# Seasandwpy/viso

Measured on AMD Instinct MI355X. Metric: stereo frames/sec at 1242x375 grey, 1/2/4/8 GPUs; pose RMSE vs reference, higher is better.
Workload: dtype f64

## Files before the change

### viso_amd/csrc/common.hpp

```cpp
#pragma once

#include <hip/hip_runtime.h>

#include <cstddef>
#include <cstdint>
#include <cstdio>

namespace viso {

constexpr int kLevels = 4;
constexpr int kHalfPatch = 4;
constexpr int kPatch = 64;
constexpr int kMaxWidth = 4096;

struct PyrGeom {
    int w[kLevels], h[kLevels];
    size_t off[kLevels];
    size_t bytes;
    size_t slot;
};

inline PyrGeom make_geom(int w, int h) {
    PyrGeom g{};
    size_t off = 0;
// ... 36 lines not shown
    return ((const __attribute__((address_space(1))) uint8_t*)p)[i];
}
__device__ inline uint8_t ld_global_u8_off(const uint8_t* base, uint32_t off) {
    return ((const __attribute__((address_space(1))) uint8_t*)base)[off];
}
__device__ inline int ld_u8_or0(const uint8_t* p, long long n, long long i) {
    const bool in = i >= 0 && i < n;
    const int v = ld_global_u8(p, in ? i : 0);
    return in ? v : 0;
}
__device__ inline uint8_t ld_lds_u8(const uint8_t* p, int i) {
    return ((const __attribute__((address_space(3))) uint8_t*)p)[i];
}
__device__ inline void st_lds_u8(uint8_t* p, int i, uint8_t v) {
    ((__attribute__((address_space(3))) uint8_t*)p)[i] = v;
}

__device__ inline double sample_px(const uint8_t* __restrict__ img, int w, int h, double x,
                                   double y) {
    const long long n = (long long)w * (long long)h;
    const bool finite = (x > -1e9 && x < 1e9 && y > -1e9 && y < 1e9);
    long long base = finite ? (long long)(int)y * (long long)w + (long long)(int)x : -(1LL << 40);
    double d0 = (double)ld_u8_or0(img, n, base);
    double d1 = (double)ld_u8_or0(img, n, base + 1);
    double d2 = (double)ld_u8_or0(img, n, base + w);
    double d3 = (double)ld_u8_or0(img, n, base + w + 1);
    double xx = x - floor(x);
    double yy = y - floor(y);
    return double((1 - xx) * (1 - yy) * d0 + xx * (1 - yy) * d1 + (1 - xx) * yy * d2 +
                  xx * yy * d3);
}

__device__ inline void gradient_px(const uint8_t* __restrict__ img, int w, int h, double u,
                                   double v, double& gx, double& gy) {
    gx = 0.5 * (sample_px(img, w, h, u + 1, v) - sample_px(img, w, h, u - 1, v));
    gy = 0.5 * (sample_px(img, w, h, u, v + 1) - sample_px(img, w, h, u, v - 1));
}

__device__ inline double wave_tree_sum(double v) {
#pragma unroll
    for (int off = 1; off < 64; off <<= 1) v = v + __shfl_xor(v, off, 64);
    return v;
}

template <int CTRL>
__device__ inline double dpp_f64(double v) {
    const long long b = __double_as_longlong(v);
    const int lo = __builtin_amdgcn_mov_dpp((int)(b & 0xffffffffLL), CTRL, 0xF, 0xF, true);
    const int hi = __builtin_amdgcn_mov_dpp((int)(b >> 32), CTRL, 0xF, 0xF, true);
    return __longlong_as_double(((long long)hi << 32) | (unsigned int)lo);
}

__device__ inline int wave_id() { return __builtin_amdgcn_readfirstlane((int)(threadIdx.x >> 6)); }

__device__ inline double uniform_f64(double v) {
    const long long b = __double_as_longlong(v);
    const int lo = __builtin_amdgcn_readfirstlane((int)(b & 0xffffffffLL));
    const int hi = __builtin_amdgcn_readfirstlane((int)(b >> 32));
    return __longlong_as_double(((long long)hi << 32) | (unsigned int)lo);
}

__device__ inline double readlane_f64(double v, int lane) {
    const long long b = __double_as_longlong(v);
    const int lo = __builtin_amdgcn_readlane((int)(b & 0xffffffffLL), lane);
    const int hi = __builtin_amdgcn_readlane((int)(b >> 32), lane);
    return __longlong_as_double(((long long)hi << 32) | (unsigned int)lo);
}

__device__ inline void permlane16_swap_f64(double a, double b, double& ra, double& rb) {
    const long long x = __double_as_longlong(a), y = __double_as_longlong(b);
    const auto lo = __builtin_amdgcn_permlane16_swap((unsigned)(x & 0xffffffffLL),
                                                     (unsigned)(y & 0xffffffffLL), false, false);
    const auto hi = __builtin_amdgcn_permlane16_swap((unsigned)(x >> 32), (unsigned)(y >> 32), false,
                                                     false);
    ra = __longlong_as_double(((long long)hi[0] << 32) | lo[0]);
    rb = __longlong_as_double(((long long)hi[1] << 32) | lo[1]);
}

__device__ inline void permlane32_swap_f64(double a, double b, double& ra, double& rb) {
    const long long x = __double_as_longlong(a), y = __double_as_longlong(b);
    const auto lo = __builtin_amdgcn_permlane32_swap((unsigned)(x & 0xffffffffLL),
                                                     (unsigned)(y & 0xffffffffLL), false, false);
    const auto hi = __builtin_amdgcn_permlane32_swap((unsigned)(x >> 32), (unsigned)(y >> 32), false,
                                                     false);
    ra = __longlong_as_double(((long long)hi[0] << 32) | lo[0]);
    rb = __longlong_as_double(((long long)hi[1] << 32) | lo[1]);
}

__device__ inline double wave_tree_sum_dpp(double v) {
    v = v + dpp_f64<0xB1>(v);
    v = v + dpp_f64<0x4E>(v);
    v = v + dpp_f64<0x141>(v);
    v = v + dpp_f64<0x140>(v);
    double a, b;
    permlane16_swap_f64(v, v, a, b);
    v = a + b;
    permlane32_swap_f64(v, v, a, b);
    return a + b;
}

__device__ inline double dsel(bool c, double a, double b) { return c ? a : b; }

__device__ inline void wave_tree_sum3(double a, double b, double c, double& ra, double& rb, double& rc) {
    const int lane = threadIdx.x & 63;
    const bool b0 = lane & 1, b1 = lane & 2, b2 = lane & 4, b3 = lane & 8;
    const double p = (b0 ? b : a) + dpp_f64<0xB1>(b0 ? a : b);
    const double q = (b0 ? 0.0 : c) + dpp_f64<0xB1>(b0 ? c : 0.0);
    double v = (b1 ? q : p) + dpp_f64<0x4E>(b1 ? p : q);
    const double r4 = dpp_f64<0x114>(v), l4 = dpp_f64<0x104>(v);
    v = v + dsel(b2, r4, l4);
    v = v + dpp_f64<0x128>(v);
    double x, y;
    permlane16_swap_f64(v, v, x, y);
    v = x + y;
    permlane32_swap_f64(v, v, x, y);
    v = x + y;
    ra = readlane_f64(v, 0);
    rb = readlane_f64(v, 1);
    rc = readlane_f64(v, 2);
}

__device__ inline void wave_tree_sum3_desc(double a, double b, double c, double& ra, double& rb, double& rc) {
    const int lane = threadIdx.x & 63;
    const bool b2 = lane & 4, b3 = lane & 8;
    double x, y;
    permlane32_swap_f64(a, b, x, y);
    const double ab = x + y;
    permlane32_swap_f64(c, c, x, y);
    const double cc = x + y;
    permlane16_swap_f64(ab, cc, x, y);
    double v = x + y;
    v = v + dpp_f64<0x128>(v);
    v = v + dpp_f64<0x124>(v);
    v = v + dpp_f64<0x4E>(v);
    v = v + dpp_f64<0xB1>(v);
    ra = readlane_f64(v, 0);
    rb = readlane_f64(v, 32);
    rc = readlane_f64(v, 16);
}


template <int CTRL>
__device__ inline double dpp_or0(double v) {
    return dpp_f64<CTRL>(v);
}

__device__ inline double swizzle_xor16_f64(double v) {
    const long long b = __double_as_longlong(v);
    const int lo = __builtin_amdgcn_ds_swizzle((int)(b & 0xffffffffLL), 0x401F);
    const int hi = __builtin_amdgcn_ds_swizzle((int)(b >> 32), 0x401F);
    return __longlong_as_double(((long long)hi << 32) | (unsigned int)lo);
}

__device__ inline double reduce_scatter_28(const double* v, int* value_index) {
    const int lane = threadIdx.x & 63;
    const bool b0 = lane & 1, b1 = lane & 2, b2 = lane & 4, b3 = lane & 8, b4 = lane & 16;
    double a[14];
#pragma unroll
    for (int k = 0; k < 14; ++k) {
        const double send = dsel(b0, v[k], v[14 + k]);
        const double keep = dsel(b0, v[14 + k], v[k]);
        a[k] = keep + dpp_f64<0xB1>(send);
    }
    double c[7];
#pragma unroll
    for (int k = 0; k < 7; ++k) {
        const double send = dsel(b1, a[k], a[7 + k]);
        const double keep = dsel(b1, a[7 + k], a[k]);
        c[k] = keep + dpp_f64<0x4E>(send);
    }
    double d[4];
#pragma unroll
    for (int k = 0; k < 4; ++k) {
        const double hi = k < 3 ? c[4 + k] : 0.0;
        const double send = dsel(b2, c[k], hi);
        const double keep = dsel(b2, hi, c[k]);
        const double recv = dsel(b2, dpp_f64<0x114>(send), dpp_f64<0x104>(send));
        d[k] = keep + recv;
    }
    double e[2];
#pragma unroll
    for (int k = 0; k < 2; ++k) {
        const double send = dsel(b3, d[k], d[2 + k]);
        const double keep = dsel(b3, d[2 + k], d[k]);
        const double recv = dpp_f64<0x128>(send);
        e[k] = keep + recv;
    }
    double ra, rb;
    permlane16_swap_f64(e[0], e[1], ra, rb);
    double f = ra + rb;
    permlane32_swap_f64(f, f, ra, rb);
    f = ra + rb;
    *value_index = (b0 ? 14 : 0) + (b1 ? 7 : 0) + (b2 ? 4 : 0) + (b3 ? 2 : 0) + (b4 ? 1 : 0);
    const int local = (b2 ? 4 : 0) + (b3 ? 2 : 0) + (b4 ? 1 : 0);
    if (local >= 7) *value_index = -1;
    return f;
}

__device__ inline double reduce_scatter_28_desc(const double* v, int* value_index) {
    const int lane = threadIdx.x & 63;
    const bool b0 = lane & 1, b1 = lane & 2, b2 = lane & 4, b3 = lane & 8, b4 = lane & 16, b5 = lane & 32;
    double a[14];
#pragma unroll
    for (int k = 0; k < 14; ++k) {
        double ra, rb;
        permlane32_swap_f64(v[k], v[14 + k], ra, rb);
        a[k] = ra + rb;
    }
    double c[7];
#pragma unroll
    for (int k = 0; k < 7; ++k) {
        double ra, rb;
        permlane16_swap_f64(a[k], a[7 + k], ra, rb);
        c[k] = ra + rb;
    }
    double d[4];
#pragma unroll
    for (int k = 0; k < 4; ++k) {
        const double hi = k < 3 ? c[4 + k] : 0.0;
        const double send = dsel(b3, c[k], hi);
        const double keep = dsel(b3, hi, c[k]);
        const double recv = dpp_f64<0x128>(send);
        d[k] = keep + recv;
    }
    double e[2];
#pragma unroll
    for (int k = 0; k < 2; ++k) {
        const double send = dsel(b2, d[k], d[2 + k]);
        const double keep = dsel(b2, d[2 + k], d[k]);
        const double recv = dsel(b2, dpp_f64<0x114>(send), dpp_f64<0x104>(send));
        e[k] = keep + recv;
    }
    const double send = dsel(b1, e[0], e[1]);
    const double keep = dsel(b1, e[1], e[0]);
    double f = keep + dpp_f64<0x4E>(send);
    f = f + dpp_f64<0xB1>(f);
    const int local = (b3 ? 4 : 0) + (b2 ? 2 : 0) + (b1 ? 1 : 0);
    *value_index = (b0 || local >= 7) ? -1 : (b5 ? 14 : 0) + (b4 ? 7 : 0) + local;
    return f;
}

template <int CTRL>
__device__ inline float dpp_f32(float v) {
    return __int_as_float(__builtin_amdgcn_mov_dpp(__float_as_int(v), CTRL, 0xF, 0xF, true));
}

__device__ inline void permlane16_swap_f32(float a, float b, float& ra, float& rb) {
    const auto r = __builtin_amdgcn_permlane16_swap((unsigned)__float_as_int(a), (unsigned)__float_as_int(b),
                                                    false, false);
    ra = __int_as_float((int)r[0]);
    rb = __int_as_float((int)r[1]);
}

__device__ inline void permlane32_swap_f32(float a, float b, float& ra, float& rb) {
    const auto r = __builtin_amdgcn_permlane32_swap((unsigned)__float_as_int(a), (unsigned)__float_as_int(b),
                                                    false, false);
    ra = __int_as_float((int)r[0]);
    rb = __int_as_float((int)r[1]);
}

__device__ inline float reduce_scatter_28_f32(const float* v, int* value_index) {
    const int lane = threadIdx.x & 63;
    const bool b0 = lane & 1, b1 = lane & 2, b2 = lane & 4, b3 = lane & 8, b4 = lane & 16;
    float a[14];
#pragma unroll
    for (int k = 0; k < 14; ++k) {
        const float send = b0 ? v[k] : v[14 + k];
        const float keep = b0 ? v[14 + k] : v[k];
        a[k] = keep + dpp_f32<0xB1>(send);
    }
    float c[7];
#pragma unroll
    for (int k = 0; k < 7; ++k) {
        const float send = b1 ? a[k] : a[7 + k];
        const float keep = b1 ? a[7 + k] : a[k];
        c[k] = keep + dpp_f32<0x4E>(send);
    }
    float d[4];
#pragma unroll
    for (int k = 0; k < 4; ++k) {
        const float hi = k < 3 ? c[4 + k] : 0.0f;
        const float send = b2 ? c[k] : hi;
        const float keep = b2 ? hi : c[k];
        const float r4 = dpp_f32<0x114>(send), l4 = dpp_f32<0x104>(send);
        const float recv = b2 ? r4 : l4;
        d[k] = keep + recv;
    }
    float e[2];
#pragma unroll
    for (int k = 0; k < 2; ++k) {
        const float send = b3 ? d[k] : d[2 + k];
        const float keep = b3 ? d[2 + k] : d[k];
        e[k] = keep + dpp_f32<0x128>(send);
    }
    float ra, rb;
    permlane16_swap_f32(e[0], e[1], ra, rb);
    float f = ra + rb;
    permlane32_swap_f32(f, f, ra, rb);
    f = ra + rb;
    *value_index = (b0 ? 14 : 0) + (b1 ? 7 : 0) + (b2 ? 4 : 0) + (b3 ? 2 : 0) + (b4 ? 1 : 0);
    const int local = (b2 ? 4 : 0) + (b3 ? 2 : 0) + (b4 ? 1 : 0);
    if (local >= 7) *value_index = -1;
    return f;
}

__device__ inline void wave_tree_sum3_f32(float a, float b, float c, float& ra, float& rb, float& rc) {
// ... 68 lines not shown
```

### viso_amd/csrc/direct.hip

```cpp
#include <algorithm>
#include <cstring>

#include "device_math.hpp"
#include "direct_solve.hpp"
#include "kernels.hpp"

#ifdef VISO_PROBE
constexpr int kPRing = 4096;
constexpr int kPSt = 16;
__device__ unsigned long long g_plog[kPRing][kPSt];
__device__ unsigned long long g_pexit[kPRing];
constexpr int kPRingB = 512;
__device__ unsigned long long g_pblk[kPRingB][256][4];
__device__ unsigned long long g_pwave[kPRingB][256][16];
#ifdef VISO_PROBE_PT
constexpr int kPtRing = 128, kPtBlocks = 32, kPtStamps = 5;
__device__ unsigned long long g_ppt[kPtRing][kPtBlocks][16][kPtStamps];
#define PPT(k)                                                                                       \
    do {                                                                                             \
        if (blockIdx.x < kPtBlocks && (threadIdx.x & 63) == 0)                                       \
            g_ppt[a.probe_seq & (kPtRing - 1)][blockIdx.x][threadIdx.x >> 6][(k)] =                  \
                __builtin_amdgcn_s_memrealtime();                                                    \
    } while (0)
#endif
#define PROBE_DECL()                                \
    __shared__ unsigned long long pst[kPSt];        \
    const unsigned long long probe_t0 = __builtin_amdgcn_s_memrealtime()
#define PST(k)                                                                       \
    do {                                                                             \
        if (blockIdx.x == 0 && (threadIdx.x & 63) == 0) pst[(k)] = __builtin_amdgcn_s_memrealtime(); \
    } while (0)
#else
#define PROBE_DECL()
#define PST(k)
#endif
#ifndef VISO_PROBE_PT
#define PPT(k) ((void)0)
#endif

namespace viso {

namespace {

constexpr int kSums = 28;
#ifndef VISO_DIRECT_WAVES
#define VISO_DIRECT_WAVES 12
#endif
constexpr int kWaves = VISO_DIRECT_WAVES;
constexpr int kThreads = kWaves * 64;
constexpr int kRigWaves = 16;
constexpr int kRigThreads = kRigWaves * 64;
constexpr int kMaxTiles = 256;
constexpr int kMaxTile = kMaxMapPoints / kMaxTiles;

inline int map_tile(int n, int groups) {
    int t = (n + groups - 1) / groups;
    return t < 1 ? 1 : (t > kMaxTile ? kMaxTile : t);
}
constexpr int kStats = 50;
constexpr int kStateStride = 8;
constexpr int kHdrBg = 1 << 17;

struct FramePair {
    FrameDev last;
    FrameDev cur;
    const double* pose_last;
};

struct LevelPair {
    const uint8_t* last;
    const uint8_t* cur;
    const double* pose_last;
};

__device__ inline LevelPair level_pair(const FramePair& fp, int lv) {
    return LevelPair{fp.last.l[lv], fp.cur.l[lv], fp.pose_last};
}

struct DirectArgs {
    FramePair fp;
    PyrDev g;
    Intrinsics K;
    const double* points;
    int n;
    const double* pose_seed;
    int level;
    int tile;
    int n_tiles;
    int split;
    DirectScratch s;
    double* stats;
    double* pose_out;
    double* log;
    int log_index;
    double* log_host;
    double* prev_log_host;
    int merged;
    int probe_seq;
    FramePair prev;
    double* prev_pose_out;
    double* prev_log;
    int prev_log_index;
    int* ready;
    int* prev_ready;
    double* flog;
};

__device__ inline void store_frame_pose(double* dst, const double* pose, int* ready) {
#pragma unroll
    for (int k = 0; k < 12; ++k) __hip_atomic_store(dst + k, pose[k], __ATOMIC_RELAXED, __HIP_MEMORY_SCOPE_AGENT);
    if (ready) {
        asm volatile("s_waitcnt vmcnt(0)" ::: "memory");
        __hip_atomic_store(ready, 1, __ATOMIC_RELAXED, __HIP_MEMORY_SCOPE_AGENT);
    }
}

__device__ inline void log_pose(double* log, double* log_host, int index, const double* pose) {
    if (!log || index < 0) return;
    for (int k = 0; k < 12; ++k) log[12 * (size_t)index + k] = pose[k];
    if (log_host)
        for (int k = 0; k < 12; ++k)
            __hip_atomic_store(log_host + 12 * (size_t)index + k, pose[k], __ATOMIC_RELAXED, __HIP_MEMORY_SCOPE_SYSTEM);
}

__device__ inline void log_frame(double* flog, int index, const SolveLds& L) {
    if (!flog || index < 0) return;
    flog[4 * (size_t)index + 0] = (double)L.ngood;
    flog[4 * (size_t)index + 1] = L.cost;
}

__device__ inline void tile_range(const DirectArgs& a, int b, int* first, int* cnt) {
    if (a.split) {
        const int f = (int)(((long long)b * a.n) / a.n_tiles);
        *first = f;
        *cnt = (int)(((long long)(b + 1) * a.n) / a.n_tiles) - f;
    } else {
        *first = b * a.tile;
        *cnt = a.tile;
    }
}

__device__ inline void d_pixel_d_xi(const Intrinsics& K, const double* pose, const double* P,
                                    double scale, double* J) {
    double Pc[3];
    mat3_vec(pose, P, Pc);
    Pc[0] = Pc[0] + pose[9];
    Pc[1] = Pc[1] + pose[10];
    Pc[2] = Pc[2] + pose[11];
    const double x = Pc[0], y = Pc[1], z = Pc[2];
    const double fx = K.fx * scale, fy = K.fy * scale;
    const double zz = z * z, xy = x * y;
    J[0] = fx / z;
    J[1] = 0;
    J[2] = -fx * x / zz;
    J[3] = -fx * xy / zz;
    J[4] = fx + fx * x * x / zz;
    J[5] = -fx * y / z;
    J[6] = 0;
    J[7] = fy / z;
    J[8] = -fy * y / zz;
    J[9] = -fy - fy * y * y / zz;
    J[10] = fy * xy / zz;
// ... 673 lines not shown
    const double xx = uc - floor(uc), yy = vc - floor(vc);
    const double w00 = (1 - xx) * (1 - yy), w10 = xx * (1 - yy), w01 = (1 - xx) * yy, w11 = xx * yy;
    const bool shared = cls == kClsShared;
    if (valid) {
        sp.v[j][k] = q;
        if (k == 0) {
            double2* v2 = reinterpret_cast<double2*>(&sp.v[j][12]);
            v2[0] = make_double2(shared ? w00 : uc, shared ? w10 : vc);
            v2[1] = make_double2(w01, w11);
            *reinterpret_cast<int4*>(sp.cls[j]) = make_int4(cls, fu, fv, 0);
        }
    }
    __builtin_amdgcn_fence(__ATOMIC_RELEASE, "workgroup");
    if (valid && k == 0) __hip_atomic_store(&sp.ready[j], 1, __ATOMIC_RELAXED, __HIP_MEMORY_SCOPE_WORKGROUP);
}

constexpr unsigned kSrcHere = 0xffffffffu;

template <bool FAST, bool LV16 = false, int W = kWaves>
__device__ void direct_tile_pf(const DirectArgs& a, const LevelPair& fp, int lv, const double* cur_pose, int b,
                               const PfLds& pf, bool merged, double* part, int* good, double* s_pts,
                               int* s_good, int* s_cnt = nullptr, double* s_qt = nullptr,
                               unsigned src_in = kSrcHere, SpLds* sp = nullptr) {
    const int wave = wave_id(), lane = threadIdx.x & 63;
    int first, T;
    tile_range(a, b, &first, &T);
    int good_cnt = 0;
    const unsigned src_lanes = FAST ? 0u : src_in != kSrcHere ? src_in : factored_sources();
    const bool sp_on = !FAST && W == kWaves && sp && s_cnt && T > kSpPoints - kSpHelpers && T <= kSpPoints;
    if (sp_on && wave >= kSpPoints) {
        __builtin_amdgcn_s_setprio(3);
        scalar_pass(a, lv, cur_pose, pf, first, T, wave - kSpPoints, *sp);
        __builtin_amdgcn_s_setprio(1);
    }
    for (int local = wave; local < T; local += W) {
        const int i = first + local;
        double f = 0.0;
        int idx = -1;
        bool ok = false;
        if (i < a.n) {
            RefSample r;
            if (merged) {
                merged_ref(a, fp, lv, pf, local, r);
                if (!FAST) ref_finish(r);
            } else if (!FAST) {
                pf_ref(pf, local, r);
            } else {
                r.P[0] = pf.P[local][0];
                r.P[1] = pf.P[local][1];
                r.P[2] = pf.P[local][2];
                r.ur = pf.ur[local];
                r.vr = pf.vr[local];
                r.ok = pf.ok[local] != 0;
                const uint32_t t = pf.taps[local][lane];
                r.t0 = (int)(t & 0xff);
                r.t1 = (int)((t >> 8) & 0xff);
                r.t2 = (int)((t >> 16) & 0xff);
                r.t3 = (int)(t >> 24);
            }
            CurWin cw;
            cw.x0 = pf.cw[local][0];
            cw.y0 = pf.cw[local][1];
            cw.on = pf.cw[local][2] != 0;
            if (FAST) {
                float ff = 0.0f;
                if (r.ok) {
                    const uint32_t t = (uint32_t)r.t0 | ((uint32_t)r.t1 << 8) | ((uint32_t)r.t2 << 16) |
                                       ((uint32_t)r.t3 << 24);
                    const float lval = (LV16 && !merged) ? (float)pf.lv16[local][lane] : fast_lval(t, r.ur, r.vr);
                    ok = direct_point_fast(a, fp, lv, cur_pose, r.P, lval, pf.win[local], cw, &ff, &idx);
                }
                f = (double)ff;
            } else if (sp_on) {
                ok = direct_point_sp(a, fp, lv, r, pf.win[local], cw, *sp, local, &f, &idx, src_lanes);
            } else {
                ok = direct_point_rs(a, fp, lv, cur_pose, r, pf.win[local], cw, &f, &idx, src_lanes,
                                     s_qt ? s_qt + 12 * wave : nullptr);
            }
        }
        if (!ok) {
            if (lane < kSums) s_pts[local * kSums + lane] = 0.0;
        } else if ((!FAST || lane < 32) && idx >= 0) {
            s_pts[local * kSums + idx] = f;
        }
        good_cnt += ok ? 1 : 0;
    }
    if (lane == 0 && good_cnt) atomicAdd(s_good, good_cnt);
#ifdef VISO_PROBE
    if (threadIdx.x == 0 && blockIdx.x < 256) g_pblk[a.probe_seq & (kPRingB - 1)][blockIdx.x][2] = __builtin_amdgcn_s_memrealtime();
    if (lane == 0 && blockIdx.x < 256 && wave < 15)
        g_pwave[a.probe_seq & (kPRingB - 1)][blockIdx.x][wave] = __builtin_amdgcn_s_memrealtime();
#endif
    if (s_cnt && T <= 16) {
        const int nw = T < W ? T : W;
        if (wave >= nw) return;
        int prev = 0;
        if (lane == 0)
            prev = __hip_atomic_fetch_add(s_cnt, 1, __ATOMIC_ACQ_REL, __HIP_MEMORY_SCOPE_WORKGROUP);
        prev = __builtin_amdgcn_readfirstlane(prev);
        if (prev != nw - 1) return;
        __builtin_amdgcn_fence(__ATOMIC_ACQUIRE, "workgroup");
        if (lane < kSums) {
            double v[16];
#pragma unroll
            for (int j = 0; j < 16; ++j) v[j] = j < T ? s_pts[j * kSums + lane] : 0.0;
#pragma unroll
            for (int st = 1; st < 16; st <<= 1)
#pragma unroll
                for (int j = 0; j < 16; j += 2 * st) v[j] = v[j] + v[j + st];
            double r = v[0] + 0.0;
            r = r + 0.0;
            part[(size_t)lane * kMaxTiles + b] = r;
        }
        if (lane == 0) good[b] = __hip_atomic_load(s_good, __ATOMIC_RELAXED, __HIP_MEMORY_SCOPE_WORKGROUP);
#ifdef VISO_PROBE
        if (lane == 0 && blockIdx.x < 256)
            g_pwave[a.probe_seq & (kPRingB - 1)][blockIdx.x][15] = __builtin_amdgcn_s_memrealtime();
#endif
        return;
    }
    __syncthreads();
    for (int k = wave; k < kSums; k += W) {
        const double v = lane < T ? s_pts[lane * kSums + k] : 0.0;
        const double r = wave_tree_sum_dpp(v);
        if (lane == 0) part[(size_t)k * kMaxTiles + b] = r;
    }
    if (threadIdx.x == 0) good[b] = *s_good;
    __syncthreads();
}

__device__ inline void state_to_pose(const double* st, double* pose) {
    double q[4] = {st[0], st[1], st[2], st[3]};
    quat_to_matrix(q, pose);
    pose[9] = st[4];
    pose[10] = st[5];
    pose[11] = st[6];
}


__device__ inline void load_partials(const double* __restrict__ part, const int* __restrict__ good,
                                     int n_tiles, double* v, int& gg) {
    const int t = threadIdx.x;
    if (t < n_tiles) {
#pragma unroll
        for (int k = 0; k < kSums; ++k) v[k] = part[(size_t)k * kMaxTiles + t];
        gg = good[t];
    } else {
#pragma unroll
        for (int k = 0; k < kSums; ++k) v[k] = 0.0;
        gg = 0;
    }
}

__device__ inline void reduce_partials(const double* v, int gg, SolveLds& L) {
    const int t = threadIdx.x, wave = t >> 6, lane = t & 63;
    if (t < 256) {
        int idx;
        const double f = reduce_scatter_28(v, &idx);
        if (lane < 32 && idx >= 0) L.red[wave][idx] = f;
        const int g = wave_sum_int(gg);
        if (lane == 0) L.g[wave] = g;
    }
    __syncthreads();
    if (t < kSums) L.S[t] = (L.red[0][t] + L.red[1][t]) + (L.red[2][t] + L.red[3][t]);
    if (t == 0) L.ngood = (L.g[0] + L.g[1]) + (L.g[2] + L.g[3]);
    __syncthreads();
}

__device__ inline void lds_barrier() { asm volatile("s_waitcnt lgkmcnt(0)\n\ts_barrier" ::: "memory"); }

template <bool FAST>
__device__ void solve_continue(const DirectArgs& a, const FramePair& fpair, int lv, SolveLds& L,
                               double* stats, double* s_pose, double* s_pts, int* s_good, PfLds& pf) {
    const int t = threadIdx.x, wave = t >> 6;
    double* part = a.s.cont_part + (size_t)blockIdx.x * kMaxTiles * kSums;
    int* good = a.s.cont_good + (size_t)blockIdx.x * kMaxTiles;
    const LevelPair fp = level_pair(fpair, lv);
    for (int iter = 1; iter < 100 && L.cont; ++iter) {
        if (t == 0) state_to_pose(L.state, s_pose);
        __syncthreads();
        double pose[12];
#pragma unroll
        for (int k = 0; k < 12; ++k) pose[k] = s_pose[k];
        for (int b = 0; b < a.n_tiles; ++b) {
            if (t == 0) *s_good = 0;
            prefetch_tile(a, lv, b, pose, fpair.pose_last, true, wave, kWaves, pf, &fpair);
            __syncthreads();
            direct_tile_pf<FAST>(a, fp, lv, pose, b, pf, false, part, good, s_pts, s_good);
        }
        __threadfence_block();
        __syncthreads();
        double v[kSums];
        int gg = 0;
        if (t < 256) load_partials(part, good, a.n_tiles, v, gg);
        reduce_partials(v, gg, L);
        if (wave == 0) {
            if (FAST)
                solve_wave0_ldlt(L, iter, stats);
            else
                solve_wave0(L, iter, stats);
        }
        __syncthreads();
    }
}

__device__ inline void prefetch_point(const DirectArgs& a, int lv, int i, bool solve, int sl,
                                      RefSample& r, CurWin& cw) {
    ref_issue(a, level_pair(a.fp, lv), lv, i, r);
    double pred[12];
    if (!solve) {
        for (int k = 0; k < 12; ++k) pred[k] = a.pose_seed[k];
    } else {
        double sp[7];
        for (int k = 0; k < 7; ++k) sp[k] = a.s.state[sl * kStateStride + k];
        state_to_pose(sp, pred);
    }
    double up, vp;
    project_px(pred, a.K, r.P, kScale[lv], up, vp);
    win_issue(a.fp.cur.l[lv], a.g.w[lv], a.g.h[lv], up, vp, cw);
}

__device__ inline void after_solve(const DirectArgs& a, bool merged, SolveLds& L, double* s_last,
                                   double* s_pose) {
    if (merged) {
        state_to_pose(L.state, s_last);
        if (blockIdx.x == 0) {
            for (int k = 0; k < 7; ++k) a.s.state[kLevels * kStateStride + k] = L.state[k];
            if (a.prev_pose_out) store_frame_pose(a.prev_pose_out, s_last, a.prev_ready);
            log_pose(a.prev_log, a.prev_log_host, a.prev_log_index, s_last);
            log_frame(a.flog, a.prev_log_index, L);
        }
        double q[4];
        quat_from_matrix(s_last, q);
        for (int k = 0; k < 4; ++k) L.state[k] = q[k];
        L.state[4] = s_last[9];
        L.state[5] = s_last[10];
        L.state[6] = s_last[11];
    }
    state_to_pose(L.state, s_pose);
}

template <bool FAST, bool SP = false>
__global__ __launch_bounds__(kThreads, 4) void direct_level_kernel(const double* __restrict__ pre_part,
                                                                 const int* __restrict__ pre_good, int pre_hdr,
                                                                 DirectArgs a) {
    PROBE_DECL();
    __builtin_amdgcn_s_setprio(1);
    __shared__ SolveLds L;
    __shared__ double s_pose[12];
    __shared__ double s_last[12];
    __shared__ double s_pts[kMaxTile * kSums];
    __shared__ int s_good;
    __shared__ int s_cnt;
    __shared__ int s_arrive;
    __shared__ PfLds s_pf;
#ifndef VISO_NO_QT
    __shared__ __attribute__((aligned(16))) double s_qt[FAST ? 2 : kWaves * 12];
    double* const qt = FAST ? nullptr : s_qt;
#else
    double* const qt = nullptr;
#endif
    __shared__ __attribute__((aligned(16))) SpLds s_sp;
    const int lv = a.level;
    const bool merged = a.merged && lv == kLevels - 1;
    const int prev = lv + 1;
    const bool solve = prev < kLevels || merged;
    const int sl = merged ? 0 : prev;
    const int t = threadIdx.x, wave = t >> 6, lane = t & 63;
    const bool tiles = lv >= 0 && (int)blockIdx.x < a.n_tiles;
    double v[kSums];
    int gg = 0;
    if (((pre_hdr >> 16) & 1) && t < 256) load_partials(pre_part, pre_good, pre_hdr & 0xffff, v, gg);
    const bool pf_wave = !solve || (wave & 3) != 0;
    double st[7];
    if (t == 256 || (solve && tiles && pf_wave)) {
        if (!solve) {
            quat_from_matrix(a.pose_seed, st);
            st[4] = a.pose_seed[9];
            st[5] = a.pose_seed[10];
            st[6] = a.pose_seed[11];
        } else {
#pragma unroll
            for (int k = 0; k < 7; ++k) st[k] = a.s.state[sl * kStateStride + k];
        }
    }
    if (t == 0) {
        s_arrive = 0;
        s_good = 0;
        s_cnt = 0;
#ifdef VISO_PROBE
        for (int k = 0; k < kPSt; ++k) pst[k] = 0;
        pst[0] = probe_t0;
        if (blockIdx.x < 256) g_pblk[a.probe_seq & (kPRingB - 1)][blockIdx.x][0] = probe_t0;
#endif
    }
    if (SP && t >= kThreads - kSpPoints) s_sp.ready[kThreads - 1 - t] = 0;
    lds_barrier();

    if (t == 256) {
        for (int k = 0; k < 7; ++k) {
            L.state[k] = st[k];
            L.best[k] = st[k];
        }
        L.cost = 0.0;
        L.last_cost = 0.0;
        L.cont = 0;
        asm volatile("s_waitcnt lgkmcnt(0)" ::: "memory");
        atomicAdd(&s_arrive, 1);
    }
    if (solve && t < 256) {
        int idx;
        const double f = reduce_scatter_28(v, &idx);
        if (lane < 32 && idx >= 0) L.red[wave][idx] = f;
        const int g = wave_sum_int(gg);
        if (lane == 0) L.g[wave] = g;
        asm volatile("s_waitcnt lgkmcnt(0)" ::: "memory");
        if (lane == 0) atomicAdd(&s_arrive, 1);
    }
    if (wave == 0) PST(1);

    const bool solver = solve && wave == 0;
    if (tiles && pf_wave) {
        double pred[12];
        if (!solve) {
            for (int k = 0; k < 12; ++k) pred[k] = a.pose_seed[k];
        } else {
            state_to_pose(st, pred);
        }
        const int first = solve ? wave - (wave >> 2) - 1 : wave;
        const int stride = solve ? kWaves - kWaves / 4 : kWaves;
        prefetch_tile(a, lv, blockIdx.x, pred, merged ? pred : a.fp.pose_last, true, first, stride, s_pf);
#ifdef VISO_PROBE
        asm volatile("s_waitcnt vmcnt(0) lgkmcnt(0)" ::: "memory");
        if (blockIdx.x == 0 && lane == 0) atomicMax(&pst[9], __builtin_amdgcn_s_memrealtime());
#endif
    }

    if (solver) {
        __builtin_amdgcn_s_setprio(3);
        while (__hip_atomic_load(&s_arrive, __ATOMIC_RELAXED, __HIP_MEMORY_SCOPE_WORKGROUP) < 5)
            __builtin_amdgcn_s_sleep(1);
        if (lane < kSums) L.S[lane] = (L.red[0][lane] + L.red[1][lane]) + (L.red[2][lane] + L.red[3][lane]);
        if (lane == 0) L.ngood = (L.g[0] + L.g[1]) + (L.g[2] + L.g[3]);
        PST(2);
        double* stp = (a.stats && blockIdx.x == 0) ? a.stats + (size_t)kStats * sl : nullptr;
#ifdef VISO_PROBE
        unsigned long long stamps[5] = {probe_t0, probe_t0, probe_t0, probe_t0, probe_t0};
        if (FAST)
            solve_wave0_ldlt(L, 0, stp, stamps);
        else
            solve_wave0(L, 0, stp, stamps);
        if (blockIdx.x == 0 && lane == 0)
            for (int k = 0; k < 4; ++k) pst[3 + k] = stamps[k];
        if (blockIdx.x == 0 && lane == 0) pst[12] = stamps[4];
#else
        if (FAST)
            solve_wave0_ldlt(L, 0, stp);
        else
            solve_wave0(L, 0, stp);
#endif
        PST(7);
        __builtin_amdgcn_s_setprio(1);
    }
    if (!solve && wave == 0 && lane == 0) {
        while (__hip_atomic_load(&s_arrive, __ATOMIC_RELAXED, __HIP_MEMORY_SCOPE_WORKGROUP) < 1)
            __builtin_amdgcn_s_sleep(1);
    }
    if (wave == 0 && lane == 0 && !L.cont) after_solve(a, merged, L, s_last, s_pose);
    const unsigned src_lanes = FAST ? 0u : factored_sources();
    __syncthreads();
    if (__builtin_expect(solve && L.cont, 0)) {
        double* stp = (a.stats && blockIdx.x == 0) ? a.stats + (size_t)kStats * sl : nullptr;
        solve_continue<FAST>(a, merged ? a.prev : a.fp, sl, L, stp, s_pose, s_pts, &s_good, s_pf);
        if (t == 0) {
            after_solve(a, merged, L, s_last, s_pose);
            s_good = 0;
        }
        __syncthreads();
        if (tiles) {
            double pose[12];
#pragma unroll
            for (int k = 0; k < 12; ++k) pose[k] = s_pose[k];
            prefetch_tile(a, lv, blockIdx.x, pose, merged ? s_last : a.fp.pose_last, true, wave, kWaves, s_pf);
        }
        __syncthreads();
    }
    if (wave == 0) PST(8);
#ifdef VISO_PROBE
    if (t == 0 && blockIdx.x < 256) g_pblk[a.probe_seq & (kPRingB - 1)][blockIdx.x][1] = __builtin_amdgcn_s_memrealtime();
#endif
    const int out = lv >= 0 ? lv : kLevels;
    if (blockIdx.x == 0 && t == 0 && !merged) {
        for (int k = 0; k < 7; ++k) a.s.state[out * kStateStride + k] = L.state[k];
        if (lv < 0 && a.pose_out) {
            store_frame_pose(a.pose_out, s_pose, a.ready);
            log_pose(a.log, a.log_host, a.log_index, s_pose);
            log_frame(a.flog, a.log_index, L);
        }
    }
    if (blockIdx.x == 0 && t == 0 && merged)
        for (int k = 0; k < 7; ++k) a.s.state[lv * kStateStride + k] = L.state[k];
    if (tiles) {
        LevelPair fp = level_pair(a.fp, lv);
        if (merged) fp.pose_last = s_last;
        double pose[12];
#pragma unroll
        for (int k = 0; k < 12; ++k) pose[k] = s_pose[k];
        direct_tile_pf<FAST>(a, fp, lv, pose, blockIdx.x, s_pf, merged, a.s.part + (size_t)lv * kMaxTiles * kSums,
                       a.s.good + lv * kMaxTiles, s_pts, &s_good, &s_cnt, qt, src_lanes,
                       SP ? &s_sp : nullptr);
    }
#ifdef VISO_PROBE
    __syncthreads();
    const unsigned long long t_exit = __builtin_amdgcn_s_memrealtime();
    const int slot = a.probe_seq & (kPRing - 1);
    if (t == 0 && blockIdx.x < 256) g_pblk[a.probe_seq & (kPRingB - 1)][blockIdx.x][3] = t_exit;
    if (blockIdx.x == 0 && t == 0) {
        pst[11] = t_exit;
        pst[15] = (unsigned long long)(lv + 1) | ((unsigned long long)merged << 8) |
                  ((unsigned long long)a.n_tiles << 16);
        for (int k = 0; k < kPSt; ++k) g_plog[slot][k] = pst[k];
    }
#endif
}

constexpr int kRigTiles = kMaxTiles;

__device__ __host__ inline int rig_reduce_waves(int n_tiles) { return n_tiles <= 64 ? 1 : n_tiles <= 128 ? 2 : 4; }

struct RigCamArgs {
    DirectArgs d;
    const double* Ad;
    double E[12];
};

struct RigArgs {
    RigCamArgs cam[kMaxRigCams];
    int n_cams;
    int tile_off[kMaxRigCams + 1];
    int level;
    double* state;
    const double* seed;
    double* stats;
    double* pose_out;
    double* log;
    int log_index;
    double* cam_last;
    int merged;
    double* prev_pose_out;
    double* prev_log;
    int prev_log_index;
};

__device__ inline void rig_compose(const double* E, const double* T, double* out) {
#pragma unroll
    for (int i = 0; i < 3; ++i) {
#pragma unroll
        for (int j = 0; j < 3; ++j)
            out[3 * i + j] = (E[3 * i] * T[j] + E[3 * i + 1] * T[3 + j]) + E[3 * i + 2] * T[6 + j];
        out[9 + i] = ((E[3 * i] * T[9] + E[3 * i + 1] * T[10]) + E[3 * i + 2] * T[11]) + E[9 + i];
    }
}

__device__ inline int rig_camera(const RigArgs& ra, int b) {
    int c = 0;
#pragma unroll
    for (int k = 1; k < kMaxRigCams; ++k) {
        const int off = ra.tile_off[k];
        if (k < ra.n_cams && b >= off) c = k;
    }
    return c;
}

__device__ inline void rig_contrib(int q, double (*red)[kSums], const double* Ad, double* sM, double* con) {
    const int lane = threadIdx.x & 63;
    if (q > 1 && lane < kSums) {
        const double v = q == 2 ? red[0][lane] + red[1][lane]
                                : (red[0][lane] + red[1][lane]) + (red[2][lane] + red[3][lane]);
        red[0][lane] = v;
    }
    asm volatile("s_waitcnt lgkmcnt(0)" ::: "memory");
    const double* S = red[0];
    if (lane < 36) {
        const int i = lane / 6, j = lane - 6 * (lane / 6);
        double m = 0.0;
#pragma unroll
        for (int k = 0; k < 6; ++k) {
            const int a = i < k ? i : k, bb = i < k ? k : i;
            const double h = S[a * 6 - (a * (a - 1)) / 2 + (bb - a)];
            m = k == 0 ? h * Ad[j] : m + h * Ad[6 * k + j];
        }
        sM[lane] = m;
    }
    asm volatile("s_waitcnt lgkmcnt(0)" ::: "memory");
// ... 632 lines not shown
```

### viso_amd/csrc/direct_solve.hpp

```cpp
#pragma once

#include "common.hpp"
#include "device_math.hpp"


namespace viso {

constexpr int kSolveSums = 28;
constexpr int kSolveStateStride = 8;

struct SolveLds {
    double red[4][kSolveSums];
    double S[kSolveSums];
    int g[4];
    int ngood;
    double state[kSolveStateStride], best[kSolveStateStride];
    double cost, last_cost;
    int cont;
};

#define SPROBE(k)                                                   \
    do {                                                            \
        if (stamps) stamps[(k)] = __builtin_amdgcn_s_memrealtime(); \
    } while (0)

__device__ __attribute__((always_inline)) inline void solve_finish(SolveLds& L, const double* update, double h, int iter, double* stats,
                                    unsigned long long* stamps) {
    const int lane = threadIdx.x & 63;
    const bool in = lane < 36;
    const int ngood = L.ngood;
    double cost = L.cost + L.S[27];
    cost /= ngood;
    const double lastCost = L.last_cost;
    const bool nan_update = isnan(update[0]);
    const bool cost_up = iter > 0 && cost > lastCost;
    const bool converged = (1 - cost / (double)lastCost) < 0.005;
    SE3d T21;
#pragma unroll
    for (int k = 0; k < 4; ++k) T21.q[k] = L.state[k];
#pragma unroll
    for (int k = 0; k < 3; ++k) T21.t[k] = L.state[4 + k];
    SE3d E;
    {
        const double eps = 1e-10;
        const double* w = update + 3;
        const double theta_sq = (w[0] * w[0] + w[1] * w[1]) + w[2] * w[2];
        const double theta = sqrt(theta_sq);
        const double half_theta = 0.5 * theta;
        double sn, cs;
        sincos((lane & 1) ? theta : half_theta, &sn, &cs);
        const double s_half = readlane_f64(sn, 0), c_half = readlane_f64(cs, 0);
        const double s_th = readlane_f64(sn, 1), c_th = readlane_f64(cs, 1);
        double imag, real;
        if (theta < eps) {
            const double theta_po4 = theta_sq * theta_sq;
            imag = 0.5 - (1.0 / 48.0) * theta_sq + (1.0 / 3840.0) * theta_po4;
            real = 1.0 - 0.5 * theta_sq + (1.0 / 384.0) * theta_po4;
        } else {
            imag = s_half / theta;
            real = c_half;
        }
        E.q[0] = imag * w[0];
        E.q[1] = imag * w[1];
        E.q[2] = imag * w[2];
        E.q[3] = real;
        double V[9];
        if (theta < eps) {
            quat_to_matrix(E.q, V);
        } else {
            const double O[9] = {0.0, -w[2], w[1], w[2], 0.0, -w[0], -w[1], w[0], 0.0};
            double O2[9];
#pragma unroll
            for (int i = 0; i < 3; ++i)
#pragma unroll
                for (int j = 0; j < 3; ++j)
                    O2[3 * i + j] = (O[3 * i + 0] * O[0 + j] + O[3 * i + 1] * O[3 + j]) + O[3 * i + 2] * O[6 + j];
            const double th2 = theta * theta;
            const double c1 = (1.0 - c_th) / th2;
            const double c2 = (theta - s_th) / (th2 * theta);
#pragma unroll
            for (int i = 0; i < 9; ++i) {
                const double id = (i % 4 == 0) ? 1.0 : 0.0;
                V[i] = (id + c1 * O[i]) + c2 * O2[i];
            }
        }
        mat3_vec(V, update, E.t);
    }
    SPROBE(3);
    T21 = se3_mul(E, T21);
    if (stats) {
        if (in) stats[2 + lane] = h;
        if (lane == 0) {
            stats[0] = ngood;
            stats[1] = cost;
            for (int k = 0; k < 6; ++k) stats[38 + k] = L.S[21 + k];
            for (int k = 0; k < 6; ++k) stats[44 + k] = update[k];
        }
    }
    if (lane == 0) {
        int cont = 1;
        if (nan_update) {
            for (int k = 0; k < 7; ++k) L.state[k] = L.best[k];
            cont = 0;
        } else {
            for (int k = 0; k < 4; ++k) L.state[k] = T21.q[k];
            for (int k = 0; k < 3; ++k) L.state[4 + k] = T21.t[k];
            if (cost_up) {
                for (int k = 0; k < 7; ++k) L.state[k] = L.best[k];
                cont = 0;
            } else if (converged) {
                cont = 0;
            } else {
                for (int k = 0; k < 7; ++k) L.best[k] = L.state[k];
                L.last_cost = cost;
            }
        }
        L.cost = cost;
        L.cont = cont;
    }
}



__device__ __attribute__((always_inline)) inline void solve_after_lu(SolveLds& L, const double* A, const int* tr,
                                                                      double h, int iter, double* stats,
                                                                      unsigned long long* stamps);

__device__ __attribute__((always_inline)) inline void solve_wave0_rep(SolveLds& L, int iter, double* stats,
                                   unsigned long long* stamps = nullptr) {
    const int lane = threadIdx.x & 63;
    const int row = lane / 6, col = lane - 6 * (lane / 6);
    const bool in = lane < 36;
    const int r0 = row < col ? row : col, c0 = row < col ? col : row;
    const double h = in ? L.S[r0 * 6 - (r0 * (r0 - 1)) / 2 + (c0 - r0)] : 0.0;
    double A[36];
    int tr[6];
#ifdef VISO_LU_TWICE
#pragma clang loop unroll(disable)
    for (int rep = 0; rep < 2; ++rep) {
#endif
#pragma unroll
    for (int r = 0; r < 6; ++r)
#pragma unroll
        for (int c = 0; c < 6; ++c) {
            const int r1 = r < c ? r : c, c1 = r < c ? c : r;
            A[6 * r + c] = L.S[r1 * 6 - (r1 * (r1 - 1)) / 2 + (c1 - r1)];
        }
#pragma unroll
    for (int k = 0; k < 6; ++k) {
        int p = k;
        double best = fabs(A[7 * k]);
#pragma unroll
        for (int i = k + 1; i < 6; ++i) {
            const double s = fabs(A[6 * i + k]);
            if (s > best) {
                best = s;
                p = i;
            }
        }
        p = __builtin_amdgcn_readfirstlane(p);
        tr[k] = p;
        if (__builtin_amdgcn_readfirstlane(best != 0.0 ? 1 : 0)) {
#pragma unroll
            for (int i = k + 1; i < 6; ++i) {
                if (p == i) {
#pragma unroll
                    for (int c = 0; c < 6; ++c) {
                        const double tmp = A[6 * k + c];
                        A[6 * k + c] = A[6 * i + c];
                        A[6 * i + c] = tmp;
                    }
                }
            }
            const double piv = A[7 * k];
#pragma unroll
            for (int i = k + 1; i < 6; ++i) A[6 * i + k] = A[6 * i + k] / piv;
        }
#pragma unroll
        for (int i = k + 1; i < 6; ++i)
#pragma unroll
            for (int c = k + 1; c < 6; ++c) A[6 * i + c] = A[6 * i + c] - A[6 * i + k] * A[6 * k + c];
    }
#ifdef VISO_LU_TWICE
    if (rep == 0) {
        asm volatile("" ::"v"(A[35]), "v"(A[0]));
        if (stamps) stamps[4] = __builtin_amdgcn_s_memrealtime();
    }
    }
#endif
    SPROBE(0);
    solve_after_lu(L, A, tr, h, iter, stats, stamps);
}

__device__ __attribute__((always_inline)) inline void solve_after_lu(SolveLds& L, const double* A, const int* tr,
                                                                      double h, int iter, double* stats,
                                                                      unsigned long long* stamps) {
    const int lane = threadIdx.x & 63;
    const int cc = lane < 6 ? lane : 0;
    int pos = cc;
#pragma unroll
    for (int k = 0; k < 6; ++k) {
        if (pos == k) pos = tr[k];
        else if (pos == tr[k]) pos = k;
    }
    double x[6];
#pragma unroll
    for (int r = 0; r < 6; ++r) x[r] = (r == pos) ? 1.0 : 0.0;
#pragma unroll
    for (int j = 0; j < 6; ++j)
#pragma unroll
        for (int i = j + 1; i < 6; ++i) x[i] = x[i] - A[6 * i + j] * x[j];
#pragma unroll
    for (int j = 5; j >= 0; --j) {
        x[j] = x[j] / A[7 * j];
#pragma unroll
        for (int i = 0; i < j; ++i) x[i] = x[i] - A[6 * i + j] * x[j];
    }
    SPROBE(1);
    double update[6];
    {
        double* Tt = &L.red[0][0];
        if (lane < 6) {
#pragma unroll
            for (int r = 0; r < 6; ++r) Tt[6 * r + lane] = x[r];
        }
        asm volatile("s_waitcnt lgkmcnt(0)" ::: "memory");
        double s = 0.0;
        if (lane < 6) {
            const double* row = Tt + 6 * lane;
            s = row[0] * L.S[21];
#pragma unroll
            for (int c = 1; c < 6; ++c) s = s + row[c] * L.S[21 + c];
        }
#pragma unroll
        for (int r = 0; r < 6; ++r) update[r] = readlane_f64(s, r);
    }
    SPROBE(2);
    solve_finish(L, update, h, iter, stats, stamps);
}


__device__ inline double bperm_f64(double v, int src) {
    const long long b = __double_as_longlong(v);
    const int lo = __builtin_amdgcn_ds_bpermute(src * 4, (int)(b & 0xffffffffLL));
    const int hi = __builtin_amdgcn_ds_bpermute(src * 4, (int)(b >> 32));
    return __longlong_as_double(((long long)hi << 32) | (unsigned int)lo);
}

__device__ __attribute__((always_inline)) inline void solve_wave0_lane(SolveLds& L, int iter, double* stats,
                                                                        unsigned long long* stamps = nullptr) {
    const int lane = threadIdx.x & 63;
    const int r = lane / 6, c = lane - 6 * (lane / 6);
    const bool in = lane < 36;
    const int r0 = r < c ? r : c, c0 = r < c ? c : r;
    const double h = in ? L.S[r0 * 6 - (r0 * (r0 - 1)) / 2 + (c0 - r0)] : 0.0;
    double a = h;
    int tr[6];
#pragma unroll
    for (int k = 0; k < 6; ++k) {
        int p = k;
        double best = fabs(readlane_f64(a, 7 * k));
#pragma unroll
        for (int i = k + 1; i < 6; ++i) {
            const double s = fabs(readlane_f64(a, 6 * i + k));
            if (s > best) {
                best = s;
                p = i;
            }
        }
        p = __builtin_amdgcn_readfirstlane(p);
        tr[k] = p;
        if (__builtin_amdgcn_readfirstlane(best != 0.0 ? 1 : 0)) {
            if (p != k) a = bperm_f64(a, r == k ? 6 * p + c : (r == p ? 6 * k + c : lane));
            const double piv = readlane_f64(a, 7 * k);
            if (in && r > k && c == k) a = a / piv;
        }
        if (k < 5) {
            const double lk = bperm_f64(a, 6 * r + k), kc = bperm_f64(a, 6 * k + c);
            if (in && r > k && c > k) a = a - lk * kc;
        }
    }
    double* T = &L.red[0][0];
    if (in) T[lane] = a;
    asm volatile("s_waitcnt lgkmcnt(0)" ::: "memory");
    double A[36];
#pragma unroll
    for (int i = 0; i < 36; ++i) A[i] = T[i];
    asm volatile("s_waitcnt lgkmcnt(0)" ::: "memory");
    SPROBE(0);
    solve_after_lu(L, A, tr, h, iter, stats, stamps);
}


__device__ __attribute__((always_inline)) inline void solve_wave0(SolveLds& L, int iter, double* stats,
                                                                   unsigned long long* stamps = nullptr) {
#ifdef VISO_SOLVE_LANE
    solve_wave0_lane(L, iter, stats, stamps);
#else
    solve_wave0_rep(L, iter, stats, stamps);
#endif
}

__device__ __attribute__((always_inline)) inline void solve_wave0_ldlt(SolveLds& L, int iter, double* stats,
                                        unsigned long long* stamps = nullptr) {
    const int lane = threadIdx.x & 63;
    const int row = lane / 6, col = lane - 6 * (lane / 6);
    const bool in = lane < 36;
    const int r0 = row < col ? row : col, c0 = row < col ? col : row;
    const double h = in ? L.S[r0 * 6 - (r0 * (r0 - 1)) / 2 + (c0 - r0)] : 0.0;
    double A[21];
#pragma unroll
    for (int i = 0; i < 6; ++i)
#pragma unroll
        for (int j = 0; j <= i; ++j) A[i * (i + 1) / 2 + j] = L.S[j * 6 - (j * (j - 1)) / 2 + (i - j)];
    double b[6];
#pragma unroll
    for (int k = 0; k < 6; ++k) b[k] = L.S[21 + k];
    double Dinv[6];
    bool bad = false;
#pragma unroll
    for (int k = 0; k < 6; ++k) {
        double d = A[k * (k + 1) / 2 + k];
#pragma unroll
        for (int j = 0; j < k; ++j) {
            const double lkj = A[k * (k + 1) / 2 + j];
            d = __builtin_fma(-lkj * lkj, A[j * (j + 1) / 2 + j], d);
        }
        bad = bad || !(d > 0.0) || !(d < 1e300);
        const double di = 1.0 / d;
        Dinv[k] = di;
        A[k * (k + 1) / 2 + k] = d;
#pragma unroll
        for (int i = k + 1; i < 6; ++i) {
            double s = A[i * (i + 1) / 2 + k];
#pragma unroll
            for (int j = 0; j < k; ++j)
                s = __builtin_fma(-A[i * (i + 1) / 2 + j] * A[j * (j + 1) / 2 + j], A[k * (k + 1) / 2 + j], s);
            A[i * (i + 1) / 2 + k] = s * di;
        }
    }
    SPROBE(0);
    double y[6];
#pragma unroll
    for (int i = 0; i < 6; ++i) {
        double s = b[i];
#pragma unroll
        for (int j = 0; j < i; ++j) s = __builtin_fma(-A[i * (i + 1) / 2 + j], y[j], s);
        y[i] = s;
    }
    double update[6];
#pragma unroll
    for (int i = 5; i >= 0; --i) {
        double s = y[i] * Dinv[i];
#pragma unroll
        for (int j = i + 1; j < 6; ++j) s = __builtin_fma(-A[j * (j + 1) / 2 + i], update[j], s);
        update[i] = s;
    }
    if (bad)
#pragma unroll
        for (int k = 0; k < 6; ++k) update[k] = __builtin_nan("");
    SPROBE(1);
    SPROBE(2);
    solve_finish(L, update, h, iter, stats, stamps);
}

}
```

Measured before the change: 21200.

## Pair tile partials per lane and spread LU pivot divisions across lanes

```diff
diff --git a/viso_amd/csrc/common.hpp b/viso_amd/csrc/common.hpp
--- a/viso_amd/csrc/common.hpp
+++ b/viso_amd/csrc/common.hpp
@@ -212,6 +212,43 @@
     return __longlong_as_double(((long long)hi << 32) | (unsigned int)lo);
 }
 
+__device__ inline double reduce_scatter_28_paired(const double* a, int* value_index) {
+    const int lane = threadIdx.x & 63;
+    const bool b0 = lane & 1, b1 = lane & 2, b2 = lane & 4, b3 = lane & 8, b5 = lane & 32;
+    double c[7];
+#pragma unroll
+    for (int k = 0; k < 7; ++k) {
+        const double send = dsel(b0, a[k], a[7 + k]);
+        const double keep = dsel(b0, a[7 + k], a[k]);
+        c[k] = keep + dpp_f64<0xB1>(send);
+    }
+    double d[4];
+#pragma unroll
+    for (int k = 0; k < 4; ++k) {
+        const double hi = k < 3 ? c[4 + k] : 0.0;
+        const double send = dsel(b1, c[k], hi);
+        const double keep = dsel(b1, hi, c[k]);
+        d[k] = keep + dpp_f64<0x4E>(send);
+    }
+    double e[2];
+#pragma unroll
+    for (int k = 0; k < 2; ++k) {
+        const double send = dsel(b2, d[k], d[2 + k]);
+        const double keep = dsel(b2, d[2 + k], d[k]);
+        const double recv = dsel(b2, dpp_f64<0x114>(send), dpp_f64<0x104>(send));
+        e[k] = keep + recv;
+    }
+    const double send = dsel(b3, e[0], e[1]);
+    const double keep = dsel(b3, e[1], e[0]);
+    double f = keep + dpp_f64<0x128>(send);
+    double ra, rb;
+    permlane16_swap_f64(f, f, ra, rb);
+    f = ra + rb;
+    const int local = (b1 ? 4 : 0) + (b2 ? 2 : 0) + (b3 ? 1 : 0);
+    *value_index = local >= 7 ? -1 : (b5 ? 14 : 0) + (b0 ? 7 : 0) + local;
+    return f;
+}
+
 __device__ inline double reduce_scatter_28(const double* v, int* value_index) {
     const int lane = threadIdx.x & 63;
     const bool b0 = lane & 1, b1 = lane & 2, b2 = lane & 4, b3 = lane & 8, b4 = lane & 16;
diff --git a/viso_amd/csrc/direct.hip b/viso_amd/csrc/direct.hip
--- a/viso_amd/csrc/direct.hip
+++ b/viso_amd/csrc/direct.hip
@@ -7,7 +7,7 @@
 
 #ifdef VISO_PROBE
 constexpr int kPRing = 4096;
-constexpr int kPSt = 16;
+constexpr int kPSt = 24;
 __device__ unsigned long long g_plog[kPRing][kPSt];
 __device__ unsigned long long g_pexit[kPRing];
 constexpr int kPRingB = 512;
@@ -987,6 +987,26 @@
     }
 }
 
+__device__ inline void load_partials_paired(const double* __restrict__ part, const int* __restrict__ good,
+                                            int n_tiles, double* a, int& gg) {
+    const int t = threadIdx.x;
+    const int t0 = (t & ~63) + 2 * (t & 31);
+    if (t0 < n_tiles) {
+        const bool has1 = t0 + 1 < n_tiles;
+        const double2* __restrict__ p2 =
+            reinterpret_cast<const double2*>(part + ((t & 32) ? (size_t)(kSums / 2) * kMaxTiles : 0) + t0);
+#pragma unroll
+        for (int k = 0; k < kSums / 2; ++k) {
+            const double2 x = p2[(size_t)k * (kMaxTiles / 2)];
+            a[k] = x.x + (has1 ? x.y : 0.0);
+        }
+    } else {
+#pragma unroll
+        for (int k = 0; k < kSums / 2; ++k) a[k] = 0.0;
+    }
+    gg = t < n_tiles ? good[t] : 0;
+}
+
 __device__ inline void reduce_partials(const double* v, int gg, SolveLds& L) {
     const int t = threadIdx.x, wave = t >> 6, lane = t & 63;
     if (t < 256) {
@@ -1103,9 +1123,9 @@
     const int sl = merged ? 0 : prev;
     const int t = threadIdx.x, wave = t >> 6, lane = t & 63;
     const bool tiles = lv >= 0 && (int)blockIdx.x < a.n_tiles;
-    double v[kSums];
+    double v[kSums / 2];
     int gg = 0;
-    if (((pre_hdr >> 16) & 1) && t < 256) load_partials(pre_part, pre_good, pre_hdr & 0xffff, v, gg);
+    if (((pre_hdr >> 16) & 1) && t < 256) load_partials_paired(pre_part, pre_good, pre_hdr & 0xffff, v, gg);
     const bool pf_wave = !solve || (wave & 3) != 0;
     double st[7];
     if (t == 256 || (solve && tiles && pf_wave)) {
@@ -1131,6 +1151,7 @@
     }
     if (SP && t >= kThreads - kSpPoints) s_sp.ready[kThreads - 1 - t] = 0;
     lds_barrier();
+    if (wave == 0) PST(16);
 
     if (t == 256) {
         for (int k = 0; k < 7; ++k) {
@@ -1144,12 +1165,17 @@
         atomicAdd(&s_arrive, 1);
     }
     if (solve && t < 256) {
+#ifdef VISO_PROBE
+        asm volatile("s_waitcnt vmcnt(0)" ::: "memory");
+        if (wave == 0) PST(17);
+#endif
         int idx;
-        const double f = reduce_scatter_28(v, &idx);
-        if (lane < 32 && idx >= 0) L.red[wave][idx] = f;
+        const double f = reduce_scatter_28_paired(v, &idx);
+        if (!(lane & 16) && idx >= 0) L.red[wave][idx] = f;
         const int g = wave_sum_int(gg);
         if (lane == 0) L.g[wave] = g;
         asm volatile("s_waitcnt lgkmcnt(0)" ::: "memory");
+        if (wave == 0) PST(18);
         if (lane == 0) atomicAdd(&s_arrive, 1);
     }
     if (wave == 0) PST(1);
@@ -1160,6 +1186,12 @@
         if (!solve) {
             for (int k = 0; k < 12; ++k) pred[k] = a.pose_seed[k];
         } else {
+#ifdef VISO_PROBE
+            if (wave == 5) {
+                asm volatile("s_waitcnt vmcnt(0)" ::: "memory");
+                PST(20);
+            }
+#endif
             state_to_pose(st, pred);
         }
         const int first = solve ? wave - (wave >> 2) - 1 : wave;
@@ -1175,6 +1207,7 @@
         __builtin_amdgcn_s_setprio(3);
         while (__hip_atomic_load(&s_arrive, __ATOMIC_RELAXED, __HIP_MEMORY_SCOPE_WORKGROUP) < 5)
             __builtin_amdgcn_s_sleep(1);
+        PST(19);
         if (lane < kSums) L.S[lane] = (L.red[0][lane] + L.red[1][lane]) + (L.red[2][lane] + L.red[3][lane]);
         if (lane == 0) L.ngood = (L.g[0] + L.g[1]) + (L.g[2] + L.g[3]);
         PST(2);
diff --git a/viso_amd/csrc/direct_solve.hpp b/viso_amd/csrc/direct_solve.hpp
--- a/viso_amd/csrc/direct_solve.hpp
+++ b/viso_amd/csrc/direct_solve.hpp
@@ -126,6 +126,7 @@
                                                                       double h, int iter, double* stats,
                                                                       unsigned long long* stamps);
 
+template <bool QL = false>
 __device__ __attribute__((always_inline)) inline void solve_wave0_rep(SolveLds& L, int iter, double* stats,
                                    unsigned long long* stamps = nullptr) {
     const int lane = threadIdx.x & 63;
@@ -173,8 +174,17 @@
                 }
             }
             const double piv = A[7 * k];
-#pragma unroll
-            for (int i = k + 1; i < 6; ++i) A[6 * i + k] = A[6 * i + k] / piv;
+            if (QL && k < 4) {
+                double num = A[6 * (k + 1) + k];
+#pragma unroll
+                for (int i = k + 2; i < 6; ++i) num = (lane == i - k - 1) ? A[6 * i + k] : num;
+                const double q = num / piv;
+#pragma unroll
+                for (int i = k + 1; i < 6; ++i) A[6 * i + k] = readlane_f64(q, i - k - 1);
+            } else {
+#pragma unroll
+                for (int i = k + 1; i < 6; ++i) A[6 * i + k] = A[6 * i + k] / piv;
+            }
         }
 #pragma unroll
         for (int i = k + 1; i < 6; ++i)
@@ -292,12 +302,15 @@
 }
 
 
+#ifndef VISO_SOLVE_QL
+#define VISO_SOLVE_QL 1
+#endif
 __device__ __attribute__((always_inline)) inline void solve_wave0(SolveLds& L, int iter, double* stats,
                                                                    unsigned long long* stamps = nullptr) {
 #ifdef VISO_SOLVE_LANE
     solve_wave0_lane(L, iter, stats, stamps);
 #else
-    solve_wave0_rep(L, iter, stats, stamps);
+    solve_wave0_rep<VISO_SOLVE_QL>(L, iter, stats, stamps);
 #endif
 }
 
```

Measured after the change: 21670 (median of 6 runs). +2.2%, better.
